# RobotVisionHKA/LiFCal

Measured on AMD Instinct MI355X. Metric: micro-image obs/sec through Jacobian+Schur at 1M obs, higher is better.
Workload: dtype f64; 1 GPU; metric_web: 334 frames, 24720 points, 999994 micro-image observations, window 10, config 0xf06 (2 radial + tangential, mlCenterAdj, Cauchy(0.5), refine poses+points); lens_selection=reference generator (lifcal_mla_project), obs_per_gpu=999994, n_reduced=2021, deterministic=False

## Files before the change

### include/lifcal_ba.h

```cpp
#ifndef LIFCAL_BA_H
#define LIFCAL_BA_H

#include <stdint.h>
#include <stddef.h>

#ifdef __cplusplus
extern "C" {
#endif

#define LIFCAL_BA_MAX_CAMERA_PARAMETERS 17

#define LIFCAL_BA_CFG_NRADIAL_MASK   0x000003u
#define LIFCAL_BA_CFG_TANGENTIAL     0x000004u
#define LIFCAL_BA_CFG_REFINE_POSES   0x000100u
#define LIFCAL_BA_CFG_ROBUST         0x000200u
#define LIFCAL_BA_CFG_REFINE_POINTS  0x000400u
#define LIFCAL_BA_CFG_ML_CENTER_ADJ  0x000800u

typedef enum {
  LIFCAL_BA_OK               =  0,
  LIFCAL_BA_ERR_INVALID_ARG  = -1,
  LIFCAL_BA_ERR_NO_DEVICE    = -2,
  LIFCAL_BA_ERR_HIP          = -3,
  LIFCAL_BA_ERR_OUT_OF_RANGE = -4,
// ... 221 lines not shown
void lifcal_ba_destroy(lifcal_ba_handle* h);
const char* lifcal_ba_strerror(int code);
const char* lifcal_ba_last_error(void);
const char* lifcal_ba_version(void);

typedef struct lifcal_ba_plan_info {
  uint32_t n_groups, n_tiles, n_lenses, n_promoted, n_reduced, max_group_obs, n_chunks, max_window_frames;
} lifcal_ba_plan_info;
int lifcal_ba_plan(const lifcal_ba_problem* p, int32_t rank, int32_t world_size,
                   lifcal_ba_plan_info* info,
                   uint32_t* obs_order ,
                   uint32_t* point_owner );

typedef struct lifcal_ba_plan_statistics {
  uint32_t n_blocks, n_passes, pass_lanes, max_block_passes;
  uint64_t n_lanes;
  uint64_t pass_steps;
  uint64_t tile_steps;
  uint64_t n_obs_window;
  uint64_t n_points_permuted;
  uint64_t violations;
  double block_cost_mean, block_cost_max;
} lifcal_ba_plan_statistics;
int lifcal_ba_plan_stats(const lifcal_ba_problem* p, int32_t rank, int32_t world_size, lifcal_ba_plan_statistics* out);

typedef struct lifcal_ba_plan_shape_figures {
  uint64_t tiles_0_steps, tiles_1_step, tiles_2_steps, tiles_odd_steps , tiles_even_steps ;
  uint64_t ell_rows;
  uint64_t max_row_read;
  uint64_t last_tile_row0;
  uint32_t last_tile_steps;
  uint32_t min_pass_points, max_pass_points;
  uint32_t min_block_passes, max_block_passes;
  uint32_t reserved;
} lifcal_ba_plan_shape_figures;
int lifcal_ba_plan_shape(const lifcal_ba_problem* p, int32_t rank, int32_t world_size, lifcal_ba_plan_shape_figures* out);

typedef struct lifcal_ba_partition {
  uint32_t world_size, n_frames, n_points, band_width;
  uint64_t n_obs;
  int32_t*  point_owner;
  uint32_t* rank_first;
  uint32_t* rank_frames;
  uint64_t* rank_obs;
  uint8_t*  frame_used;
} lifcal_ba_partition;
int lifcal_ba_partition_points(const lifcal_ba_problem* index_only, lifcal_ba_partition* part);
int lifcal_ba_create_shard(const lifcal_ba_problem* local, const lifcal_ba_partition* part, const lifcal_ba_options* o, lifcal_ba_handle** out);
int lifcal_ba_plan_shard(const lifcal_ba_problem* local, const lifcal_ba_partition* part, int32_t rank, lifcal_ba_plan_info* info);

typedef struct lifcal_init_problem {
  uint64_t n;
  const double* vdepth;
  const uint32_t* fr;
  const uint32_t* pt;
  uint32_t n_frames, n_points;
  const double* world_to_cam;
  const double* pts;
  double fL_init;
} lifcal_init_problem;
typedef struct lifcal_init_result {
  double B_init, bL0_init;
  uint64_t n_used;
  int32_t rank;
  int32_t reserved;
} lifcal_init_result;
int lifcal_init_plenoptic(const lifcal_init_problem* p, int32_t device, lifcal_init_result* out);
int lifcal_init_plenoptic_recalibration(double fL_fixed, double B_fixed, lifcal_init_result* out);

// ... 5 lines not shown
```

### lifcal_amd/__init__.py

```python
from . import _capi, scene
from .bundle_adjustment import (BundleAdjustment, Covariance, LifcalError, make_config, plan, plan_stats, plan_shape, comm_unique_id, initPlenopticParameters,
                                performBundleAdjustmentWindowed, GroupTable, ResidualReport, sensor_cells, check_priors, prior_from_covariance,
                                check_point_priors, alignFit, alignApply, alignScene, Alignment)
from .mla import MicroLensGrid, RawObservations
from .depth import DepthMaps, backProjectPoints, projectPoints, readDepthData, read_png16, depth_is_estimable
from .resection import resectFrames, ResectionResult
from .intersection import intersectPoints, IntersectionResult
from .start import startPoses, startPoints, StartPosesResult, StartPointsResult
from .register import registerScene, RegisterResult
from .grid_fit import detectLensCentres, fitGridCentres, fitGrid, GridFit, GridReport
```

### lifcal_amd/_capi.py

```python
from __future__ import annotations

import ctypes as C
import os

import numpy as np

_HERE = os.path.dirname(os.path.abspath(__file__))
LIB_PATH = os.environ.get("LIFCAL_BA_LIB") or os.path.join(_HERE, "csrc", "liblifcal_ba.so")

dptr = C.POINTER(C.c_double)
uptr = C.POINTER(C.c_uint32)


class Problem(C.Structure):
    _fields_ = [
        ("n_obs", C.c_uint32), ("n_frames", C.c_uint32), ("n_points", C.c_uint32), ("n_constraints", C.c_uint32),
        ("u", dptr), ("v", dptr), ("mcx", dptr), ("mcy", dptr), ("pt", uptr), ("fr", uptr),
        ("cam", dptr), ("views", dptr), ("pts", dptr),
        ("spx", C.c_double), ("spy", C.c_double), ("scale", C.c_double),
        ("config", C.c_uint32), ("fixed_mask", C.c_uint32),
        ("lower", dptr), ("upper", dptr),
        ("c_i", uptr), ("c_j", uptr), ("c_dist", dptr), ("c_sigma", dptr),
        ("use_constraints", C.c_uint32), ("reserved", C.c_uint32),
    ]
# ... 81 lines not shown
        F, P = problem.struct.n_frames, problem.struct.n_points
        self.point_owner = np.zeros(max(P, 1), np.int32); self.rank_first = np.zeros(world_size, np.uint32); self.rank_frames = np.zeros(world_size, np.uint32)
        self.rank_obs = np.zeros(world_size, np.uint64); self.frame_used = np.zeros(max(F, 1), np.uint8)
        self.struct = Partition(world_size, 0, 0, 0, 0, self.point_owner.ctypes.data_as(C.POINTER(C.c_int32)), as_uptr(self.rank_first), as_uptr(self.rank_frames),
                                self.rank_obs.ctypes.data_as(C.POINTER(C.c_uint64)), self.frame_used.ctypes.data_as(C.POINTER(C.c_uint8)))
        rc = lib.lifcal_ba_partition_points(C.byref(problem.struct), C.byref(self.struct))
        if rc:
            raise RuntimeError(f"lifcal_ba_partition_points: {rc}")

    def shard_of(self, problem: "ProblemArrays", rank: int) -> "ProblemArrays":
        sel = np.flatnonzero(self.point_owner[problem.pt] == rank)
        return ProblemArrays(problem.u[sel], problem.v[sel], problem.mcx[sel], problem.mcy[sel], problem.pt[sel], problem.fr[sel], problem.cam, problem.views, problem.pts,
                             problem.struct.spx, problem.struct.scale, problem.struct.config, spy=problem.struct.spy, fixed_mask=problem.struct.fixed_mask,
                             lower=problem.lower, upper=problem.upper, use_constraints=0)


class PlanInfo(C.Structure):
    _fields_ = [("n_groups", C.c_uint32), ("n_tiles", C.c_uint32), ("n_lenses", C.c_uint32), ("n_promoted", C.c_uint32),
                ("n_reduced", C.c_uint32), ("max_group_obs", C.c_uint32), ("n_chunks", C.c_uint32),
                ("max_window_frames", C.c_uint32)]


class PlanStats(C.Structure):
    _fields_ = [("n_blocks", C.c_uint32), ("n_passes", C.c_uint32), ("pass_lanes", C.c_uint32), ("max_block_passes", C.c_uint32),
                ("n_lanes", C.c_uint64), ("pass_steps", C.c_uint64), ("tile_steps", C.c_uint64), ("n_obs_window", C.c_uint64),
                ("n_points_permuted", C.c_uint64), ("violations", C.c_uint64),
                ("block_cost_mean", C.c_double), ("block_cost_max", C.c_double)]


class PlanShape(C.Structure):
    _fields_ = [("tiles_0_steps", C.c_uint64), ("tiles_1_step", C.c_uint64), ("tiles_2_steps", C.c_uint64), ("tiles_odd_steps", C.c_uint64),
                ("tiles_even_steps", C.c_uint64), ("ell_rows", C.c_uint64), ("max_row_read", C.c_uint64), ("last_tile_row0", C.c_uint64),
                ("last_tile_steps", C.c_uint32), ("min_pass_points", C.c_uint32), ("max_pass_points", C.c_uint32),
                ("min_block_passes", C.c_uint32), ("max_block_passes", C.c_uint32), ("reserved", C.c_uint32)]


ALLREDUCE_FN =C.CFUNCTYPE(C.c_int, C.c_void_p, C.c_void_p, C.c_size_t, C.c_void_p)
ALLGATHER_FN = C.CFUNCTYPE(C.c_int, C.c_void_p, C.c_void_p, C.c_void_p, C.c_size_t, C.c_void_p)

class InitProblem(C.Structure):
    _fields_ = [("n", C.c_uint64), ("vdepth", C.POINTER(C.c_double)), ("fr", C.POINTER(C.c_uint32)), ("pt", C.POINTER(C.c_uint32)),
                ("n_frames", C.c_uint32), ("n_points", C.c_uint32), ("world_to_cam", C.POINTER(C.c_double)), ("pts", C.POINTER(C.c_double)),
                ("fL_init", C.c_double)]


class InitResult(C.Structure):
    _fields_ = [("B_init", C.c_double), ("bL0_init", C.c_double), ("n_used", C.c_uint64), ("rank", C.c_int32), ("reserved", C.c_int32)]


class InitArrays:

    def __init__(self, vdepth, fr, pt, world_to_cam, pts, fL_init):
        self.vdepth = np.ascontiguousarray(vdepth, np.float64)
        self.fr = np.ascontiguousarray(fr, np.uint32)
        self.pt = np.ascontiguousarray(pt, np.uint32)
        w = np.asarray(world_to_cam, np.float64).reshape(-1, 4, 4)
        self.w2c = np.ascontiguousarray(np.transpose(w, (0, 2, 1)).reshape(-1, 16))
        self.pts = np.ascontiguousarray(np.asarray(pts, np.float64).reshape(-1, 3))
        assert len(self.vdepth) == len(self.fr) == len(self.pt)
        self.struct = InitProblem(len(self.vdepth), as_dptr(self.vdepth), as_uptr(self.fr), as_uptr(self.pt), len(self.w2c), len(self.pts),
                                  as_dptr(self.w2c), as_dptr(self.pts), float(fL_init))


class MlaParams(C.Structure):
    _fields_ = [("width", C.c_int32), ("height", C.c_int32), ("lens_diameter", C.c_float), ("lens_base_y", C.c_float * 2),
                ("rotation", C.c_float), ("offset", C.c_float * 2), ("rotation_on_grid", C.c_int32)]

# ... 361 lines not shown
    "lifcal_ba_create": (C.c_int, [C.POINTER(Problem), C.POINTER(Options), C.POINTER(C.c_void_p)]),
    "lifcal_ba_solve": (C.c_int, [C.c_void_p, C.POINTER(Summary)]),
    "lifcal_ba_sweep": (C.c_int, [C.c_void_p, C.c_double, C.POINTER(SweepOut)]),
    "lifcal_ba_sweep_enqueue": (C.c_int, [C.c_void_p, C.c_double]),
    "lifcal_ba_profile_begin": (C.c_int, [C.c_void_p, C.c_uint32]),
    "lifcal_ba_profile_begin_sampled": (C.c_int, [C.c_void_p, C.c_uint32, C.c_uint32]),
    "lifcal_ba_profile_end": (C.c_int, [C.c_void_p, C.POINTER(Profile)]),
    "lifcal_ba_reproj_stats": (C.c_int, [C.c_void_p, C.c_double, C.POINTER(Stats)]),
    "lifcal_ba_project_observations": (C.c_int, [C.c_void_p, dptr, dptr]),
    "lifcal_ba_set_fixed_frames": (C.c_int, [C.c_void_p, C.POINTER(C.c_uint8)]),
    "lifcal_ba_default_covariance_options": (None, [C.POINTER(CovarianceOptions)]),
    "lifcal_ba_covariance": (C.c_int, [C.c_void_p, C.POINTER(CovarianceOptions), C.POINTER(CovarianceOut)]),
    "lifcal_ba_residual_report": (C.c_int, [C.c_void_p, C.POINTER(ResidualReportIO)]),
    "lifcal_ba_residual_groups": (C.c_int, [C.c_void_p, C.c_double, C.c_uint32, uptr, C.c_void_p]),
    "lifcal_ba_object_space_stats": (C.c_int, [C.c_void_p, C.c_uint64, dptr, dptr, dptr, uptr, uptr, dptr, dptr, C.POINTER(ObjectSpace)]),
    "lifcal_ba_solve_windowed": (C.c_int, [C.POINTER(Problem), C.POINTER(Options), C.c_uint32, C.c_uint32, C.c_void_p, C.POINTER(WindowReport), C.POINTER(C.c_uint32)]),
    "lifcal_ba_upload_parameters": (C.c_int, [C.c_void_p]),
    "lifcal_ba_download_parameters": (C.c_int, [C.c_void_p]),
    "lifcal_ba_set_allreduce": (C.c_int, [C.c_void_p, ALLREDUCE_FN, C.c_void_p]),
    "lifcal_ba_set_allgather": (C.c_int, [C.c_void_p, ALLGATHER_FN, C.c_void_p]),
    "lifcal_ba_comm_unique_id": (C.c_int, [C.c_void_p]),
    "lifcal_ba_comm_init_rccl": (C.c_int, [C.c_void_p, C.c_void_p]),
    "lifcal_ba_get_info": (C.c_int, [C.c_void_p, C.POINTER(Info)]),
    "lifcal_ba_debug_step": (C.c_int, [C.c_void_p, C.POINTER(StepOut)]),
    "lifcal_ba_destroy": (None, [C.c_void_p]),
    "lifcal_init_plenoptic": (C.c_int, [C.POINTER(InitProblem), C.c_int32, C.POINTER(InitResult)]),
    "lifcal_init_plenoptic_recalibration": (C.c_int, [C.c_double, C.c_double, C.POINTER(InitResult)]),
    "lifcal_ba_strerror": (C.c_char_p, [C.c_int]),
    "lifcal_ba_last_error": (C.c_char_p, []),
    "lifcal_ba_version": (C.c_char_p, []),
    "lifcal_ba_plan": (C.c_int, [C.POINTER(Problem), C.c_int32, C.c_int32, C.POINTER(PlanInfo), uptr, uptr]),
    "lifcal_ba_plan_stats": (C.c_int, [C.POINTER(Problem), C.c_int32, C.c_int32, C.POINTER(PlanStats)]),
    "lifcal_ba_plan_shape": (C.c_int, [C.POINTER(Problem), C.c_int32, C.c_int32, C.POINTER(PlanShape)]),
    "lifcal_ba_partition_points": (C.c_int, [C.POINTER(Problem), C.POINTER(Partition)]),
    "lifcal_ba_create_shard": (C.c_int, [C.POINTER(Problem), C.POINTER(Partition), C.POINTER(Options), C.POINTER(C.c_void_p)]),
    "lifcal_ba_plan_shard": (C.c_int, [C.POINTER(Problem), C.POINTER(Partition), C.c_int32, C.POINTER(PlanInfo)]),
}

HOST_PROTOTYPES = {
    "lifcal_group_index": (C.c_int, [C.c_uint32, C.c_uint32, uptr, uptr, uptr]),
}

_lib = None


def load_library(path: str = LIB_PATH) -> C.CDLL:
    global _lib
    if _lib is None:
        if not os.path.exists(path):
            raise RuntimeError(
                f"lifcal_amd: native library {path} is missing. Build it with "
                "`python -c 'import __graft_entry__ as g; g.build()'` (hipcc --offload-arch=gfx950). "
                "There is no CPU fallback for the bundle-adjustment path.")
        lib = C.CDLL(path)
        for name, (res, args) in list(PROTOTYPES.items()) + list(MLA_PROTOTYPES.items()) + list(IO_PROTOTYPES.items()) + list(COLMAP_PROTOTYPES.items()) + list(DEPTH_PROTOTYPES.items()) + list(HOST_PROTOTYPES.items()) + list(RESECT_PROTOTYPES.items()) + list(INTERSECT_PROTOTYPES.items()) + list(START_PROTOTYPES.items()) + list(REGISTER_PROTOTYPES.items()) + list(PRIOR_PROTOTYPES.items()) + list(ALIGN_PROTOTYPES.items()) + list(GRID_PROTOTYPES.items()):
            fn = getattr(lib, name)
            fn.restype = res
            fn.argtypes = args
        _lib = lib
    return _lib


def as_dptr(a: np.ndarray):
    return a.ctypes.data_as(dptr) if a is not None else None


# ... 79 lines not shown
```

### lifcal_amd/bundle_adjustment.py

```python
from __future__ import annotations

import ctypes as C
from dataclasses import dataclass
from typing import Optional

import numpy as np

from . import _capi as capi


def make_config(nRadialDistParam=2, tangentialDistParam=True, refinePoses=True, useRobustCostFunction=True,
                refine3Dpoints=True, mlCenterAdjustment=True) -> int:
    cfg = min(int(nRadialDistParam), 2) & 0x3
    if tangentialDistParam:
        cfg |= 0x004
    if refinePoses:
        cfg |= 0x100
    if useRobustCostFunction:
        cfg |= 0x200
    if refine3Dpoints:
        cfg |= 0x400
    if mlCenterAdjustment:
        cfg |= 0x800
    return cfg
# ... 514 lines not shown
    _check(lib, lib.lifcal_ba_comm_unique_id(buf), "lifcal_ba_comm_unique_id")
    return buf.raw


def initPlenopticParameters(vdepth, fr, pt, world_to_cam, pts, fL_init, device: int = 0):
    lib = capi.load_library()
    arrs = capi.InitArrays(vdepth, fr, pt, world_to_cam, pts, fL_init)
    res = capi.InitResult()
    _check(lib, lib.lifcal_init_plenoptic(C.byref(arrs.struct), int(device), C.byref(res)), "lifcal_init_plenoptic")
    return res


def plan(problem: capi.ProblemArrays, rank: int = 0, world_size: int = 1):
    lib = capi.load_library()
    info = capi.PlanInfo()
    order = np.zeros(max(problem.struct.n_obs, 1), np.uint32)
    owner = np.zeros(max(problem.struct.n_points, 1), np.uint32)
    _check(lib, lib.lifcal_ba_plan(C.byref(problem.struct), rank, world_size, C.byref(info), capi.as_uptr(order), capi.as_uptr(owner)), "lifcal_ba_plan")
    return info, order[: problem.struct.n_obs], owner[: problem.struct.n_points].astype(np.int32)


def plan_stats(problem: capi.ProblemArrays, rank: int = 0, world_size: int = 1) -> capi.PlanStats:
    lib = capi.load_library()
    st = capi.PlanStats()
    _check(lib, lib.lifcal_ba_plan_stats(C.byref(problem.struct), rank, world_size, C.byref(st)), "lifcal_ba_plan_stats")
    return st


def plan_shape(problem: capi.ProblemArrays, rank: int = 0, world_size: int = 1) -> capi.PlanShape:
    lib = capi.load_library()
    sh = capi.PlanShape()
    _check(lib, lib.lifcal_ba_plan_shape(C.byref(problem.struct), rank, world_size, C.byref(sh)), "lifcal_ba_plan_shape")
    return sh
```

### lifcal_amd/csrc/lifcal_ba.hip

```cpp
#include <hip/hip_runtime.h>
#include <hip/hip_ext.h>

#include <dlfcn.h>

#include <chrono>
#include <cmath>
#include <cstdio>
#include <cstdlib>
#include <cstring>
#include <limits>
#include <mutex>
#include <string>
#include <vector>

#include "../../include/lifcal_ba.h"
#include "../../include/lifcal_prior.h"
#include "../../include/lifcal_align.h"
#include "kernels.hpp"
#include "point_priors.hpp"
#include "plan.hpp"
#include "linesearch.hpp"
#include "sweep_state.hpp"

using namespace lifcal;
// ... 764 lines not shown

static void fill_plan_info(const Plan& pl, lifcal_ba_plan_info* info) {
  info->n_groups = pl.n_pairs; info->n_lenses = pl.n_lenses; info->n_promoted = pl.Q;
  info->n_reduced = pl.n_red_canon; info->max_group_obs = pl.max_group_obs; info->n_chunks = pl.n_blocks; info->max_window_frames = pl.bw + 1;
  info->n_tiles = pl.n_tiles + pl.pass_tiles() * pl.n_passes;
}

int lifcal_ba_plan(const lifcal_ba_problem* p, int32_t rank, int32_t world_size, lifcal_ba_plan_info* info,
                   uint32_t* obs_order, uint32_t* point_owner) {
  Plan pl; PlanChoice c;
  if (int rc = plan_for_environment(p, rank, world_size, 0, 0, nullptr, &pl, &c)) return rc;
  if (info) fill_plan_info(pl, info);
  if (obs_order) { for (uint32_t i = 0; i < p->n_obs; ++i) obs_order[i] = UINT32_MAX; for (size_t s = 0; s < pl.obs_order.size(); ++s) obs_order[s] = pl.obs_order[s]; }
  if (point_owner) for (uint32_t q = 0; q < p->n_points; ++q) point_owner[q] = (uint32_t)pl.owner[q];
  return 0;
}

int lifcal_ba_plan_stats(const lifcal_ba_problem* p, int32_t rank, int32_t world_size, lifcal_ba_plan_statistics* out) {
  if (!out) return LIFCAL_BA_ERR_INVALID_ARG;
  Plan pl; PlanChoice c;
  if (int rc = plan_for_environment(p, rank, world_size, 0, 0, nullptr, &pl, &c)) return rc;
  plan_stats(pl, out);
  return 0;
}

int lifcal_ba_plan_shape(const lifcal_ba_problem* p, int32_t rank, int32_t world_size, lifcal_ba_plan_shape_figures* out) {
  if (!out) return LIFCAL_BA_ERR_INVALID_ARG;
  Plan pl; PlanChoice c;
  if (int rc = plan_for_environment(p, rank, world_size, 0, 0, nullptr, &pl, &c)) return rc;
  plan_shape(pl, out);
  return 0;
}

static int create_impl(const lifcal_ba_problem* p, const lifcal_ba_options* o, lifcal_ba_handle** out, const lifcal_ba_partition* part, const lifcal_ba_point_priors* pp = nullptr);

int lifcal_ba_create(const lifcal_ba_problem* p, const lifcal_ba_options* o, lifcal_ba_handle** out) { return create_impl(p, o, out, nullptr); }

int lifcal_ba_create_with_point_priors(const lifcal_ba_problem* p, const lifcal_ba_point_priors* pp, const lifcal_ba_options* o, lifcal_ba_handle** out) {
  if (!pp || pp->n == 0) {
    const int rc = create_impl(p, o, out, nullptr);
    if (!rc) (*out)->pp_entry = true;
    return rc;
  }
  if (!p || !out) return LIFCAL_BA_ERR_INVALID_ARG;
  if (o && o->world_size > 1) { g_last_error = "lifcal_ba_create_with_point_priors: world_size > 1 is not supported (every rank would add the term)"; return LIFCAL_BA_ERR_INVALID_ARG; }
  if (int rc = lifcal_ba_check_point_priors(p->n_points, pp)) return rc;
  return create_impl(p, o, out, nullptr, pp);
}

int lifcal_ba_create_shard(const lifcal_ba_problem* local, const lifcal_ba_partition* part, const lifcal_ba_options* o, lifcal_ba_handle** out) {
  if (!part) return LIFCAL_BA_ERR_INVALID_ARG;
  return create_impl(local, o, out, part);
}

int lifcal_ba_partition_points(const lifcal_ba_problem* index_only, lifcal_ba_partition* part) { return partition_points(index_only, part); }

int lifcal_ba_plan_shard(const lifcal_ba_problem* local, const lifcal_ba_partition* part, int32_t rank, lifcal_ba_plan_info* info) {
  if (!part || !info) return LIFCAL_BA_ERR_INVALID_ARG;
  Plan pl; PlanChoice c;
  if (int rc = plan_for_environment(local, rank, (int)part->world_size, 0, 0, part, &pl, &c)) return rc;
  fill_plan_info(pl, info);
  return 0;
}

static int create_impl(const lifcal_ba_problem* p, const lifcal_ba_options* o, lifcal_ba_handle** out, const lifcal_ba_partition* part, const lifcal_ba_point_priors* pp) {
  if (!out) return LIFCAL_BA_ERR_INVALID_ARG;
// ... 686 lines not shown
```

### lifcal_amd/csrc/plan.hpp

```cpp
#pragma once
#include <chrono>
#include <cstdio>
#include <cstdlib>
#include <algorithm>
#include <cstdint>
#include <cstring>
#include <numeric>
#include <atomic>
#include <new>
#include <thread>
#include <unordered_map>
#include <vector>

#include "../../include/lifcal_ba.h"

namespace lifcal {

template <class T>
struct LazyZeroAlloc {
  using value_type = T;
  LazyZeroAlloc() = default;
  template <class U> LazyZeroAlloc(const LazyZeroAlloc<U>&) {}
  T* allocate(size_t n) { void* q = std::calloc(n ? n : 1, sizeof(T)); if (!q) throw std::bad_alloc(); return (T*)q; }
  void deallocate(T* q, size_t) { std::free(q); }
// ... 820 lines not shown
        if (lanes != k) ++bad;
        ++lanes; lane_obs += n;
        const uint32_t gi = L.v2_gidx[at], fr = L.v2f_fr[at];
        if (gi < gid0 || gi >= gid0 + ng) { ++bad; continue; }
        if (seen[gi - gid0]) ++bad;
        seen[gi - gid0] = 1;
        if (gid_pt[gi] != L.v2f_pt[at] || L.gid_fr[gi] != fr || fr < L.blk_flo[b] || fr - L.blk_flo[b] >= L.blk_nf[b]) ++bad;
        if (L.frame_order && lanes > 1 && fr < prev_fr) ++bad;
        prev_fr = fr;
      }
      if (lanes != ng) ++bad;
    }
  }
  std::vector<uint8_t> owned(L.P, 0);
  for (uint32_t q : L.owned_points) owned[q] = 1;
  for (uint32_t q = 0; q < L.P; ++q) {
    const bool regular = owned[q] && !L.pt_special[q] && L.pt_nslots[q] > 0;
    if (in_pass[q] != (regular ? 1u : 0u)) ++bad;
  }
  if (lane_obs != L.n_obs_v2) ++bad;
  s.violations = bad;
  *out = s;
}

inline void plan_shape(const Plan& L, lifcal_ba_plan_shape_figures* out) {
  lifcal_ba_plan_shape_figures s;
  std::memset(&s, 0, sizeof(s));
  const uint32_t PT = L.pass_tiles();
  s.min_pass_points = s.min_block_passes = UINT32_MAX;
  s.ell_rows = L.v2_lens.size() / 64;
  for (uint32_t b = 0; b < L.n_blocks; ++b) {
    const uint32_t n = L.blk_pass0[b + 1] - L.blk_pass0[b];
    s.min_block_passes = std::min(s.min_block_passes, n); s.max_block_passes = std::max(s.max_block_passes, n);
  }
  for (uint32_t ps = 0; ps < L.n_passes; ++ps) {
    s.min_pass_points = std::min(s.min_pass_points, L.pass_np[ps]); s.max_pass_points = std::max(s.max_pass_points, L.pass_np[ps]);
    for (uint32_t w = 0; w < PT; ++w) {
      const uint32_t row0 = L.v2_tile_row0[(size_t)ps * PT + w], r = L.v2_tile_row0[(size_t)ps * PT + w + 1] - row0;
      if (r == 0) ++s.tiles_0_steps; else if (r == 1) ++s.tiles_1_step; else if (r == 2) ++s.tiles_2_steps; else if (r & 1u) ++s.tiles_odd_steps; else ++s.tiles_even_steps;
      s.max_row_read = std::max<uint64_t>(s.max_row_read, (uint64_t)row0 + std::max(r, 1u) - 1);
      if (ps + 1 == L.n_passes && w + 1 == PT) { s.last_tile_steps = r; s.last_tile_row0 = row0; }
    }
  }
  if (L.n_passes == 0) s.min_pass_points = 0;
  if (L.n_blocks == 0) s.min_block_passes = 0;
  *out = s;
}

inline int partition_points(const lifcal_ba_problem* p, lifcal_ba_partition* out) {
  if (!p || !out || out->world_size < 1 || out->world_size > 64 || !out->point_owner || !out->rank_first || !out->rank_frames || !out->rank_obs || !out->frame_used) return LIFCAL_BA_ERR_INVALID_ARG;
  if (p->n_obs && (!p->pt || !p->fr)) return LIFCAL_BA_ERR_INVALID_ARG;
  const uint32_t P = p->n_points, F = p->n_frames, N = p->n_obs, W = out->world_size;
  for (uint32_t i = 0; i < N; ++i) if (p->pt[i] >= P || p->fr[i] >= F) return LIFCAL_BA_ERR_OUT_OF_RANGE;
  std::vector<uint32_t> first(P, UINT32_MAX), last(P, 0), cnt(P, 0);
  for (uint32_t f = 0; f < F; ++f) out->frame_used[f] = 0;
  for (uint32_t i = 0; i < N; ++i) { const uint32_t q = p->pt[i], f = p->fr[i]; first[q] = std::min(first[q], f); last[q] = std::max(last[q], f); cnt[q]++; out->frame_used[f] = 1; }
  uint32_t bw = 0;
  for (uint32_t q = 0; q < P; ++q) if (cnt[q]) bw = std::max(bw, last[q] - first[q]);
  std::vector<uint32_t> order(P);
  std::iota(order.begin(), order.end(), 0u);
  std::stable_sort(order.begin(), order.end(), [&](uint32_t a, uint32_t b) { return first[a] < first[b]; });
  uint64_t acc = 0;
  std::vector<uint32_t> lo(W, UINT32_MAX), hi(W, 0);
  for (uint32_t r = 0; r < W; ++r) out->rank_obs[r] = 0;
  for (uint32_t r = 0; r < P; ++r) {
    const uint32_t q = order[r];
// ... 15 lines not shown
```

### lifcal_amd/csrc/sweep3.hpp

```cpp
#pragma once

namespace lifcal {

template <int NR, bool TAN, bool ADJ, int WR, class ET = double>
__global__ __launch_bounds__(128 * WR, 2) void k_sweep3(Dev d, double radius, int mode) {
  constexpr bool F32 = sizeof(ET) == 4;
  constexpr int NC = 5 + NR + (TAN ? 2 : 0);
  constexpr int NCC = NC * (NC + 1) / 2;
  constexpr int HV = 6 + 2 * NC + 2;
  constexpr uint32_t LP = 64u * WR;
  constexpr uint32_t NT = 2u * LP;
  static_assert(HV * LP <= V2Lds::zd_for(LP), "hand-off buffer must fit the Z matrix");
  if (radius < 0.0 && d.lm[LM_TERMINATION] != 0.0) return;
  extern __shared__ __attribute__((aligned(16))) double sm[];
  const V2Lds lay(d.v2_nfmax, true, LP);
  const uint32_t NFm = lay.nfm, vlen = 6 * NFm + NCMAX + 3;
  double* Spp = sm; double* Scp = sm + lay.off_cp; double* Scc = sm + lay.off_cc;
  double* vgB = sm + lay.off_vec; double* vhd = vgB + vlen; double* vrhs = vhd + vlen;
  double* Fr = sm + lay.off_fr;
  double* slab = sm + lay.off_slab;
  double* Zd = sm + lay.off_zd;
  double* misc = sm + lay.off_misc;
  uint32_t* pidl = (uint32_t*)(misc + MISC_DOUBLES);
  unsigned short* colinfo = (unsigned short*)(misc + MISC_DOUBLES + 32);
  uint32_t flip = 0;
#ifndef LIFCAL_NO_ROLE_FLIP
  if (WR == 2) flip = (__builtin_amdgcn_s_getreg(6 | (0 << 6) | (7 << 11)) != 0) ? LP : 0u;
#endif
  const uint32_t tid = threadIdx.x ^ flip, lane = tid & 63u, w = tid >> 6;
  const bool role_b = w >= (uint32_t)WR;
  const uint32_t wl = w & (uint32_t)(WR - 1);
  const uint32_t t256 = tid & (LP - 1u);
  const uint32_t b = blockIdx.x;
  const uint32_t flo = d.blk_flo[b], nf = d.blk_nf[b];
  const uint32_t ncol = 6 * nf + NC + 1, ncolp = (ncol + 15u) & ~15u;
  const uint32_t zs = ncolp + 2;
  const CamConsts c = *d.camc;
#ifdef LIFCAL_STAMPS
  unsigned long long st_acc[16] = {0, 0, 0, 0, 0, 0, 0, 0, 0, 0, 0, 0, 0, 0, 0, 0}, st_last = 0;
  if (tid == 0 || tid == LP) { asm volatile("s_memtime %0\n\ts_waitcnt lgkmcnt(0)" : "=s"(st_last) :: "memory"); }
#define STAMPB(i) do { if (tid == LP) { unsigned long long t_; asm volatile("s_memtime %0\n\ts_waitcnt lgkmcnt(0)" : "=s"(t_) :: "memory"); st_acc[i] += t_ - st_last; st_last = t_; } } while (0)
#else
#define STAMPB(i) do { } while (0)
#endif
  const uint32_t ps_begin = d.blk_pass0[b], ps_end = d.blk_pass0[b + 1];
  uint32_t nx_np = 0, nx_si = 0, nx_pt = 0, nx_fp = 0, nx_gid = 0, nx_r[2] = {0, 0};
  uint32_t vz;
  asm volatile("v_mov_b32 %0, 0" : "=v"(vz));
  auto fetch_pass = [&](uint32_t q) {
    nx_np = d.pass_np[q + vz];
    nx_si = d.v2_slot[(size_t)q * LP + t256]; nx_pt = d.v2f_pt[(size_t)q * LP + t256]; nx_gid = d.v2_gidx[(size_t)q * LP + t256];
    nx_r[0] = d.v2_tile_row0[q * WR + wl + vz]; nx_r[1] = d.v2_tile_row0[q * WR + wl + 1 + vz];
    nx_fp = d.v2_passpt[(size_t)q * 64 + (tid & 63u)];
  };
  if (ps_begin < ps_end) fetch_pass(ps_begin);
  { double2* z2 = reinterpret_cast<double2*>(sm); for (uint32_t i = tid; i < lay.off_slab / 2; i += NT) z2[i] = double2{0.0, 0.0}; }
  if (tid == 0 && (lay.off_slab & 1u)) sm[lay.off_slab - 1] = 0.0;
  if (tid < MISC_DOUBLES) misc[tid] = 0.0;
  for (uint32_t cI = tid; cI < ncolp; cI += NT)
    colinfo[cI] = (cI < 6 * nf) ? (unsigned short)(((cI / 6) << 8) | (cI % 6)) : (cI < ncol - 1 ? (unsigned short)(0x8000u | (cI - 6 * nf)) : (unsigned short)0xC000u);

  auto zero_slab = [&]() { for (uint32_t i = tid; i < lay.np_max * SLAB_STRIDE; i += NT) slab[i] = 0.0; };
  auto zero_zd = [&](uint32_t krows) { double2* z2 = reinterpret_cast<double2*>(Zd); for (uint32_t i = tid; i < (krows * zs) / 2; i += NT) z2[i] = double2{0.0, 0.0}; };
  auto z_phase = [&](uint32_t np) {
    const uint32_t nwc = ncol - 1;
    const uint32_t nth = NT / nwc > 0 ? NT / nwc : 1;
    const uint32_t gi = tid / nwc, cidx = tid - gi * nwc;
    if (gi < nth || nwc > NT) {
      for (uint32_t cc0 = cidx; cc0 < nwc; cc0 += (nwc > NT ? NT : nwc * nth)) {
#pragma unroll 4
        for (uint32_t lp = (nwc > NT ? 0 : gi); lp < np; lp += (nwc > NT ? 1 : nth)) {
          const double* acc = slab + lp * SLAB_STRIDE;
          double* z = Zd + (size_t)(3 * lp) * zs + cc0;
          const double w0 = z[0], w1 = z[zs], w2 = z[2 * zs];
          if (cc0 >= 6 * nf) {
            double* ga = d.ptacc + (size_t)pidl[lp] * 36 + 9 + (cc0 - 6 * nf);
            store_stream(ga, w0); store_stream(ga + NCMAX, w1); store_stream(ga + 2 * NCMAX, w2);
          }
          z[0] = acc[0] * w0; z[zs] = acc[1] * w0 + acc[3] * w1; z[2 * zs] = acc[2] * w0 + acc[4] * w1 + acc[5] * w2;
        }
      }
    }
  };
  struct LaneGeom { double R[9], Y[3], Gr[3][3]; };
  auto lane_geom = [&](uint32_t fr, uint32_t pt, LaneGeom& q) {
    const double* ft = d.ft + (size_t)fr * FRAME_STRIDE;
    const double* P = d.pts + 3 * (size_t)pt;
#pragma unroll
    for (int k = 0; k < 9; ++k) q.R[k] = ft[k];
    const double P0 = P[0], P1 = P[1], P2 = P[2];
#pragma unroll
    for (int k = 0; k < 3; ++k) q.Y[k] = q.R[3 * k] * P0 + q.R[3 * k + 1] * P1 + q.R[3 * k + 2] * P2;
    const double c0 = ft[12], s0 = ft[13], n0 = q.R[2], n1 = q.R[5], n2 = q.R[8];
    q.Gr[0][0] = 0.0;     q.Gr[0][1] = c0 * q.Y[2] - s0 * q.Y[1]; q.Gr[0][2] = n1 * q.Y[2] - n2 * q.Y[1];
    q.Gr[1][0] = -q.Y[2]; q.Gr[1][1] = s0 * q.Y[0];               q.Gr[1][2] = n2 * q.Y[0] - n0 * q.Y[2];
    q.Gr[2][0] = q.Y[1];  q.Gr[2][1] = -c0 * q.Y[0];              q.Gr[2][2] = n0 * q.Y[1] - n1 * q.Y[0];
  };
  const uint32_t frs = NFm * lay.nrep;
  struct RunMask { double m1, m2, m4, m8; bool head; };
  auto run_masks = [&](uint32_t cnt, uint32_t lf) {
    const int key = cnt > 0 ? (int)lf : (int)(0x7F000000u + lane);
    RunMask r;
    r.m1 = __builtin_amdgcn_update_dpp(-1, key, 0x101, 0xf, 0xf, false) == key ? 1.0 : 0.0;
    r.m2 = __builtin_amdgcn_update_dpp(-1, key, 0x102, 0xf, 0xf, false) == key ? 1.0 : 0.0;
    r.m4 = __builtin_amdgcn_update_dpp(-1, key, 0x104, 0xf, 0xf, false) == key ? 1.0 : 0.0;
    r.m8 = __builtin_amdgcn_update_dpp(-1, key, 0x108, 0xf, 0xf, false) == key ? 1.0 : 0.0;
    r.head = cnt > 0 && __builtin_amdgcn_update_dpp(-1, key, 0x111, 0xf, 0xf, false) != key;
    return r;
  };
  auto run_sum = [](double v, const RunMask& r) {
    auto shl = [](double x, auto ctrl) {
      const int lo = __double2loint(x), hi = __double2hiint(x);
      return __hiloint2double(__builtin_amdgcn_update_dpp(0, hi, decltype(ctrl)::value, 0xf, 0xf, true),
                              __builtin_amdgcn_update_dpp(0, lo, decltype(ctrl)::value, 0xf, 0xf, true));
    };
// ... 256 lines not shown
        }
        if (mode == 0) {
          { double* ga = d.Av + (size_t)gidx * 6;
            store_stream(ga, A[0], A[1]); store_stream(ga + 2, A[2], A[3]); store_stream(ga + 4, A[4], A[5]); }
#pragma unroll
          for (int i = 0; i < 3; ++i) {
            atomicAdd(acc + 6 + i, R[i] * bv[0] + R[3 + i] * bv[1] + R[6 + i] * bv[2]);
            double* zrow = Zd + (size_t)(3 * lp + i) * zs + 6 * lf;
            double w6[6];
#pragma unroll
            for (int j = 0; j < 3; ++j) { w6[j] = R[i] * AG[0][j] + R[3 + i] * AG[1][j] + R[6 + i] * AG[2][j]; w6[3 + j] = R[i] * Am[0][j] + R[3 + i] * Am[1][j] + R[6 + i] * Am[2][j]; }
            const bool rot = (lp & 1u) != 0;
#pragma unroll
            for (int jj = 0; jj < 6; ++jj) {
              const double wv = rot ? w6[(jj + 1) % 6] : w6[jj];
              const uint32_t col = rot ? (uint32_t)((jj + 1) % 6) : (uint32_t)jj;
              if (fpose) atomicAdd(zrow + col, wv);
            }
          }
        }
      }
      if (det) { publish(turn, my_turn + 1); my_turn += (uint32_t)WR; }
      STAMP(6);
      asm volatile("s_waitcnt lgkmcnt(0)" ::: "memory");
      if (lane == 0) __hip_atomic_fetch_add(eval_done, 1u, __ATOMIC_RELAXED, __HIP_MEMORY_SCOPE_WORKGROUP);
      ++passes_done;
      if (w == 0) wait_for(eval_done, (uint32_t)WR * passes_done);
      STAMP(1);
      if (tid < np) {
        const uint32_t p = fp;
        pidl[tid] = p;
        double* acc = slab + tid * SLAB_STRIDE;
        double U0 = acc[0], U1 = acc[1], U2 = acc[2], U3 = acc[3], U4 = acc[4], U5 = acc[5];
        if (mode == 1) {
          double* ga = d.ptacc + (size_t)p * 36;
          store_stream(ga, U0); store_stream(ga + 3, U3); store_stream(ga + 5, U5);
        } else {
          const double g0 = acc[6], g1 = acc[7], g2 = acc[8];
          double lam[3];
          {
            const double h[3] = {U0, U3, U5}, sgv[3] = {fsg0, fsg1, fsg2};
#pragma unroll
            for (int k = 0; k < 3; ++k) { const double sg = sgv[k]; lam[k] = fmin(fmax(h[k] * sg * sg, d.lm_min), d.lm_max) / (lm_radius(d, radius) * sg * sg); }
          }
          U0 += lam[0]; U3 += lam[1]; U5 += lam[2];
          bool ok = U0 > 0.0;
          double i00 = rsqrt(U0);
          const double l10 = U1 * i00, l20 = U2 * i00;
          const double d11 = U3 - l10 * l10; ok = ok && (d11 > 0.0);
          double i11 = rsqrt(d11);
          const double l21 = (U4 - l20 * l10) * i11;
          const double d22 = U5 - l20 * l20 - l21 * l21; ok = ok && (d22 > 0.0);
          double i22 = rsqrt(d22);
          double m10 = -l10 * i00 * i11, m21 = -l21 * i11 * i22, m20 = -(l20 * i00 + l21 * m10) * i22;
          if (!ok) { i00 = i11 = i22 = m10 = m21 = m20 = 0.0; atomicAdd(misc + 1, 1.0); }
          double* gu = d.Uinv + 9 * (size_t)p;
          const double v00 = i00 * i00 + m10 * m10 + m20 * m20, v01 = m10 * i11 + m20 * m21, v02 = m20 * i22;
          const double v11 = i11 * i11 + m21 * m21, v12 = m21 * i22, v22 = i22 * i22;
          {
            const double vu[9] = {v00, v01, v02, v01, v11, v12, v02, v12, v22};
#pragma unroll
            for (int k = 0; k < 9; ++k) store_stream(gu + k, vu[k]);
          }
          double* gl = d.lamP + 3 * (size_t)p;
          double* ga = d.ptacc + (size_t)p * 36 + 6;
#pragma unroll
          for (int k = 0; k < 3; ++k) store_stream(gl + k, lam[k]);
          store_stream(ga, g0); store_stream(ga + 1, g1); store_stream(ga + 2, g2);
          const double gm = fmax(fabs(g0), fmax(fabs(g1), fabs(g2)));
          atomicMax((unsigned long long*)(misc + 2), (unsigned long long)__double_as_longlong(gm));
          acc[0] = i00; acc[1] = m10; acc[2] = m20; acc[3] = i11; acc[4] = m21; acc[5] = i22;
          double* z0 = Zd + (size_t)(3 * tid) * zs + (ncol - 1);
          z0[0] = i00 * g0; z0[zs] = m10 * g0 + i11 * g1; z0[2 * zs] = m20 * g0 + m21 * g1 + i22 * g2;
        }
      }
      lds_barrier();
// ... 311 lines not shown
```

Measured before the change: 10.08 billion obs/s.

## Flatten Z-phase into point/column-pair work items with batched rounds

Replaces the nested per-column, per-point loop in z_phase with a flat item space. Each item is a (point, column pair) found by a fixed-point reciprocal division, and up to three rounds per thread are unrolled so that all loads are issued before the streaming stores and the double2 writes. This is meant to balance work across threads and raise memory-level parallelism. It also hoists lm_radius out of the per-point loop, loads g0..g2 early, and adds a host helper plus a plan statistic to check item counts. The cost is more registers per thread and reliance on the exactness of the reciprocal mapping.

```diff
diff --git a/include/lifcal_ba.h b/include/lifcal_ba.h
--- a/include/lifcal_ba.h
+++ b/include/lifcal_ba.h
@@ -277,9 +277,12 @@
   uint32_t last_tile_steps;
   uint32_t min_pass_points, max_pass_points;
   uint32_t min_block_passes, max_block_passes;
-  uint32_t reserved;
+  uint32_t max_z_items;
 } lifcal_ba_plan_shape_figures;
 int lifcal_ba_plan_shape(const lifcal_ba_problem* p, int32_t rank, int32_t world_size, lifcal_ba_plan_shape_figures* out);
+
+int lifcal_ba_zphase_items(uint32_t nf, uint32_t nc, uint32_t np, uint32_t nt, uint32_t capacity, uint32_t* point, uint32_t* first_col,
+                           uint32_t* n_items, uint32_t* rounds, uint32_t* max_rounds);
 
 typedef struct lifcal_ba_partition {
   uint32_t world_size, n_frames, n_points, band_width;
diff --git a/lifcal_amd/__init__.py b/lifcal_amd/__init__.py
--- a/lifcal_amd/__init__.py
+++ b/lifcal_amd/__init__.py
@@ -1,5 +1,5 @@
 from . import _capi, scene
-from .bundle_adjustment import (BundleAdjustment, Covariance, LifcalError, make_config, plan, plan_stats, plan_shape, comm_unique_id, initPlenopticParameters,
+from .bundle_adjustment import (BundleAdjustment, Covariance, LifcalError, make_config, plan, plan_stats, plan_shape, zphase_items, comm_unique_id, initPlenopticParameters,
                                 performBundleAdjustmentWindowed, GroupTable, ResidualReport, sensor_cells, check_priors, prior_from_covariance,
                                 check_point_priors, alignFit, alignApply, alignScene, Alignment)
 from .mla import MicroLensGrid, RawObservations
diff --git a/lifcal_amd/_capi.py b/lifcal_amd/_capi.py
--- a/lifcal_amd/_capi.py
+++ b/lifcal_amd/_capi.py
@@ -137,7 +137,7 @@
     _fields_ = [("tiles_0_steps", C.c_uint64), ("tiles_1_step", C.c_uint64), ("tiles_2_steps", C.c_uint64), ("tiles_odd_steps", C.c_uint64),
                 ("tiles_even_steps", C.c_uint64), ("ell_rows", C.c_uint64), ("max_row_read", C.c_uint64), ("last_tile_row0", C.c_uint64),
                 ("last_tile_steps", C.c_uint32), ("min_pass_points", C.c_uint32), ("max_pass_points", C.c_uint32),
-                ("min_block_passes", C.c_uint32), ("max_block_passes", C.c_uint32), ("reserved", C.c_uint32)]
+                ("min_block_passes", C.c_uint32), ("max_block_passes", C.c_uint32), ("max_z_items", C.c_uint32)]
 
 
 ALLREDUCE_FN =C.CFUNCTYPE(C.c_int, C.c_void_p, C.c_void_p, C.c_size_t, C.c_void_p)
@@ -565,6 +565,8 @@
     "lifcal_ba_plan": (C.c_int, [C.POINTER(Problem), C.c_int32, C.c_int32, C.POINTER(PlanInfo), uptr, uptr]),
     "lifcal_ba_plan_stats": (C.c_int, [C.POINTER(Problem), C.c_int32, C.c_int32, C.POINTER(PlanStats)]),
     "lifcal_ba_plan_shape": (C.c_int, [C.POINTER(Problem), C.c_int32, C.c_int32, C.POINTER(PlanShape)]),
+    "lifcal_ba_zphase_items": (C.c_int, [C.c_uint32, C.c_uint32, C.c_uint32, C.c_uint32, C.c_uint32, C.POINTER(C.c_uint32), C.POINTER(C.c_uint32),
+                               C.POINTER(C.c_uint32), C.POINTER(C.c_uint32), C.POINTER(C.c_uint32)]),
     "lifcal_ba_partition_points": (C.c_int, [C.POINTER(Problem), C.POINTER(Partition)]),
     "lifcal_ba_create_shard": (C.c_int, [C.POINTER(Problem), C.POINTER(Partition), C.POINTER(Options), C.POINTER(C.c_void_p)]),
     "lifcal_ba_plan_shard": (C.c_int, [C.POINTER(Problem), C.POINTER(Partition), C.c_int32, C.POINTER(PlanInfo)]),
diff --git a/lifcal_amd/bundle_adjustment.py b/lifcal_amd/bundle_adjustment.py
--- a/lifcal_amd/bundle_adjustment.py
+++ b/lifcal_amd/bundle_adjustment.py
@@ -570,3 +570,14 @@
     sh = capi.PlanShape()
     _check(lib, lib.lifcal_ba_plan_shape(C.byref(problem.struct), rank, world_size, C.byref(sh)), "lifcal_ba_plan_shape")
     return sh
+
+
+def zphase_items(nf: int, nc: int, n_points: int, threads: int):
+    lib = capi.load_library()
+    cap = n_points * ((6 * nf + nc + 1) // 2)
+    point = np.zeros(max(cap, 1), np.uint32)
+    col = np.zeros(max(cap, 1), np.uint32)
+    n, rounds, max_rounds = C.c_uint32(), C.c_uint32(), C.c_uint32()
+    _check(lib, lib.lifcal_ba_zphase_items(nf, nc, n_points, threads, cap, capi.as_uptr(point), capi.as_uptr(col),
+                                           C.byref(n), C.byref(rounds), C.byref(max_rounds)), "lifcal_ba_zphase_items")
+    return point[: n.value], col[: n.value], rounds.value, max_rounds.value
diff --git a/lifcal_amd/csrc/lifcal_ba.hip b/lifcal_amd/csrc/lifcal_ba.hip
--- a/lifcal_amd/csrc/lifcal_ba.hip
+++ b/lifcal_amd/csrc/lifcal_ba.hip
@@ -820,6 +820,17 @@
   return 0;
 }
 
+int lifcal_ba_zphase_items(uint32_t nf, uint32_t nc, uint32_t np, uint32_t nt, uint32_t capacity, uint32_t* point, uint32_t* first_col,
+                           uint32_t* n_items, uint32_t* rounds, uint32_t* max_rounds) {
+  if (!point || !first_col || !n_items || !rounds || !max_rounds) return LIFCAL_BA_ERR_INVALID_ARG;
+  if (nf < 1 || nf > Plan::NF_MAX || nc < 5 || nc > (uint32_t)NCMAX || np < 1 || np > Plan::NP_MAX || (nt != 512 && nt != 256)) return LIFCAL_BA_ERR_INVALID_ARG;
+  const uint32_t npair = (6 * nf + nc + 1u) >> 1, items = np * npair, recip = zmap_recip(npair);
+  if (items > capacity) return LIFCAL_BA_ERR_INVALID_ARG;
+  for (uint32_t i = 0; i < items; ++i) { point[i] = zmap_point(i, recip); first_col[i] = 2u * (i - point[i] * npair); }
+  *n_items = items; *rounds = (items + nt - 1) / nt; *max_rounds = zrounds_max(V2Lds::zd_for(nt / 2), nt);
+  return 0;
+}
+
 static int create_impl(const lifcal_ba_problem* p, const lifcal_ba_options* o, lifcal_ba_handle** out, const lifcal_ba_partition* part, const lifcal_ba_point_priors* pp = nullptr);
 
 int lifcal_ba_create(const lifcal_ba_problem* p, const lifcal_ba_options* o, lifcal_ba_handle** out) { return create_impl(p, o, out, nullptr); }
diff --git a/lifcal_amd/csrc/plan.hpp b/lifcal_amd/csrc/plan.hpp
--- a/lifcal_amd/csrc/plan.hpp
+++ b/lifcal_amd/csrc/plan.hpp
@@ -876,6 +876,8 @@
   for (uint32_t b = 0; b < L.n_blocks; ++b) {
     const uint32_t n = L.blk_pass0[b + 1] - L.blk_pass0[b];
     s.min_block_passes = std::min(s.min_block_passes, n); s.max_block_passes = std::max(s.max_block_passes, n);
+    const uint32_t npair = (6 * L.blk_nf[b] + (uint32_t)L.nc + 1u) / 2;
+    for (uint32_t ps = L.blk_pass0[b]; ps < L.blk_pass0[b + 1]; ++ps) s.max_z_items = std::max(s.max_z_items, L.pass_np[ps] * npair);
   }
   for (uint32_t ps = 0; ps < L.n_passes; ++ps) {
     s.min_pass_points = std::min(s.min_pass_points, L.pass_np[ps]); s.max_pass_points = std::max(s.max_pass_points, L.pass_np[ps]);
diff --git a/lifcal_amd/csrc/sweep3.hpp b/lifcal_amd/csrc/sweep3.hpp
--- a/lifcal_amd/csrc/sweep3.hpp
+++ b/lifcal_amd/csrc/sweep3.hpp
@@ -1,6 +1,14 @@
 #pragma once
 
 namespace lifcal {
+
+constexpr uint32_t ZMAP_SHIFT = 20;
+__host__ __device__ constexpr uint32_t zmap_recip(uint32_t npair) { return ((1u << ZMAP_SHIFT) + npair - 1u) / npair; }
+__host__ __device__ constexpr uint32_t zmap_point(uint32_t item, uint32_t recip) { return (item * recip) >> ZMAP_SHIFT; }
+__host__ __device__ constexpr bool zmap_exact(uint32_t items, uint32_t npair_max) {
+  return (uint64_t)items * (npair_max - 1u) < (1ull << ZMAP_SHIFT) && ((uint64_t)items << ZMAP_SHIFT) <= 0xFFFFFFFFull;
+}
+__host__ __device__ constexpr uint32_t zrounds_max(uint32_t zd, uint32_t nt) { return (zd / 6 + nt - 1u) / nt; }
 
 template <int NR, bool TAN, bool ADJ, int WR, class ET = double>
 __global__ __launch_bounds__(128 * WR, 2) void k_sweep3(Dev d, double radius, int mode) {
@@ -12,6 +20,7 @@
   constexpr uint32_t NT = 2u * LP;
   static_assert(HV * LP <= V2Lds::zd_for(LP), "hand-off buffer must fit the Z matrix");
   if (radius < 0.0 && d.lm[LM_TERMINATION] != 0.0) return;
+  const double lm_rad = lm_radius(d, radius);
   extern __shared__ __attribute__((aligned(16))) double sm[];
   const V2Lds lay(d.v2_nfmax, true, LP);
   const uint32_t NFm = lay.nfm, vlen = 6 * NFm + NCMAX + 3;
@@ -62,25 +71,56 @@
 
   auto zero_slab = [&]() { for (uint32_t i = tid; i < lay.np_max * SLAB_STRIDE; i += NT) slab[i] = 0.0; };
   auto zero_zd = [&](uint32_t krows) { double2* z2 = reinterpret_cast<double2*>(Zd); for (uint32_t i = tid; i < (krows * zs) / 2; i += NT) z2[i] = double2{0.0, 0.0}; };
+  const uint32_t z_nwc = ncol - 1, z_npair = (z_nwc + 1u) >> 1, z_recip = zmap_recip(z_npair);
+  auto z_rounds = [&](uint32_t nitems, auto rounds) {
+    constexpr int RN = decltype(rounds)::value;
+    double2 wv[RN][3]; double li[RN][6]; uint32_t pid[RN], c0[RN]; double* zr[RN]; bool on[RN];
+#pragma unroll
+    for (int r = 0; r < RN; ++r) {
+      const uint32_t it = tid + (uint32_t)r * NT;
+      on[r] = it < nitems;
+      const uint32_t ic = on[r] ? it : nitems - 1u;
+      const uint32_t lp = zmap_point(ic, z_recip);
+      c0[r] = 2u * (ic - lp * z_npair);
+      zr[r] = Zd + (size_t)(3 * lp) * zs + c0[r];
+      const double* acc = slab + lp * SLAB_STRIDE;
+#pragma unroll
+      for (int k = 0; k < 3; ++k) wv[r][k] = *reinterpret_cast<const double2*>(zr[r] + (size_t)k * zs);
+#pragma unroll
+      for (int k = 0; k < 6; ++k) li[r][k] = acc[k];
+      pid[r] = pidl[lp];
+    }
+#pragma unroll
+    for (int r = 0; r < RN; ++r) {
+      const bool two = c0[r] + 1u < z_nwc;
+      if (on[r] && c0[r] >= 6 * nf) {
+        double* ga = d.ptacc + (size_t)pid[r] * 36 + 9 + (c0[r] - 6 * nf);
+        store_stream(ga, wv[r][0].x); store_stream(ga + NCMAX, wv[r][1].x); store_stream(ga + 2 * NCMAX, wv[r][2].x);
+        if (two) { store_stream(ga + 1, wv[r][0].y); store_stream(ga + NCMAX + 1, wv[r][1].y); store_stream(ga + 2 * NCMAX + 1, wv[r][2].y); }
+      }
+    }
+#pragma unroll
+    for (int r = 0; r < RN; ++r) {
+      const bool two = c0[r] + 1u < z_nwc;
+      const double* a = li[r];
+      const double2 w0 = wv[r][0], w1 = wv[r][1], w2 = wv[r][2];
+      double2 q0, q1, q2;
+      q0.x = a[0] * w0.x; q1.x = a[1] * w0.x + a[3] * w1.x; q2.x = a[2] * w0.x + a[4] * w1.x + a[5] * w2.x;
+      q0.y = a[0] * w0.y; q1.y = a[1] * w0.y + a[3] * w1.y; q2.y = a[2] * w0.y + a[4] * w1.y + a[5] * w2.y;
+      if (!two) { q0.y = w0.y; q1.y = w1.y; q2.y = w2.y; }
+      if (on[r]) {
+        *reinterpret_cast<double2*>(zr[r]) = q0; *reinterpret_cast<double2*>(zr[r] + zs) = q1; *reinterpret_cast<double2*>(zr[r] + 2 * (size_t)zs) = q2;
+      }
+    }
+  };
   auto z_phase = [&](uint32_t np) {
-    const uint32_t nwc = ncol - 1;
-    const uint32_t nth = NT / nwc > 0 ? NT / nwc : 1;
-    const uint32_t gi = tid / nwc, cidx = tid - gi * nwc;
-    if (gi < nth || nwc > NT) {
-      for (uint32_t cc0 = cidx; cc0 < nwc; cc0 += (nwc > NT ? NT : nwc * nth)) {
-#pragma unroll 4
-        for (uint32_t lp = (nwc > NT ? 0 : gi); lp < np; lp += (nwc > NT ? 1 : nth)) {
-          const double* acc = slab + lp * SLAB_STRIDE;
-          double* z = Zd + (size_t)(3 * lp) * zs + cc0;
-          const double w0 = z[0], w1 = z[zs], w2 = z[2 * zs];
-          if (cc0 >= 6 * nf) {
-            double* ga = d.ptacc + (size_t)pidl[lp] * 36 + 9 + (cc0 - 6 * nf);
-            store_stream(ga, w0); store_stream(ga + NCMAX, w1); store_stream(ga + 2 * NCMAX, w2);
-          }
-          z[0] = acc[0] * w0; z[zs] = acc[1] * w0 + acc[3] * w1; z[2 * zs] = acc[2] * w0 + acc[4] * w1 + acc[5] * w2;
-        }
-      }
-    }
+    static_assert(zmap_exact(zrounds_max(V2Lds::zd_for(LP), NT) * NT, (6 * DET_NF_MAX + NCMAX + 1) / 2), "zmap_point is exact for every item of a pass");
+    static_assert(zrounds_max(V2Lds::zd_for(LP), NT) <= 3, "rounds of z_phase");
+    const uint32_t nitems = np * z_npair;
+    if (nitems == 0) return;
+    if (nitems <= NT) z_rounds(nitems, std::integral_constant<int, 1>{});
+    else if (nitems <= 2 * NT) z_rounds(nitems, std::integral_constant<int, 2>{});
+    else z_rounds(nitems, std::integral_constant<int, 3>{});
   };
   struct LaneGeom { double R[9], Y[3], Gr[3][3]; };
   auto lane_geom = [&](uint32_t fr, uint32_t pt, LaneGeom& q) {
@@ -403,16 +443,17 @@
         pidl[tid] = p;
         double* acc = slab + tid * SLAB_STRIDE;
         double U0 = acc[0], U1 = acc[1], U2 = acc[2], U3 = acc[3], U4 = acc[4], U5 = acc[5];
+        const double g0 = acc[6], g1 = acc[7], g2 = acc[8];
+        asm volatile("" ::: "memory");
         if (mode == 1) {
           double* ga = d.ptacc + (size_t)p * 36;
           store_stream(ga, U0); store_stream(ga + 3, U3); store_stream(ga + 5, U5);
         } else {
-          const double g0 = acc[6], g1 = acc[7], g2 = acc[8];
           double lam[3];
           {
             const double h[3] = {U0, U3, U5}, sgv[3] = {fsg0, fsg1, fsg2};
 #pragma unroll
-            for (int k = 0; k < 3; ++k) { const double sg = sgv[k]; lam[k] = fmin(fmax(h[k] * sg * sg, d.lm_min), d.lm_max) / (lm_radius(d, radius) * sg * sg); }
+            for (int k = 0; k < 3; ++k) { const double sg = sgv[k]; lam[k] = fmin(fmax(h[k] * sg * sg, d.lm_min), d.lm_max) / (lm_rad * sg * sg); }
           }
           U0 += lam[0]; U3 += lam[1]; U5 += lam[2];
           bool ok = U0 > 0.0;
```

Result: no change. 10.18 billion obs/s, median of 6 (+1.0%).
